# OPPO-Mente-Lab/PEA-Diffusion

Hardware: AMD Instinct MI355X
Metric: training images/sec (SDXL 1024px bf16, adapter-only bwd) (higher is better)
Workload: dtype bf16

## Files before the change

### pea_diffusion_amd/csrc/api_ops.hip

```cpp
#include <stdarg.h>
#include <string.h>

#include "../../include/pea_hip.h"
#include "pea_kernels.h"

static thread_local char g_err[512] = "";
void pea_set_error(const char* fmt, ...) {
  va_list ap;
  va_start(ap, fmt);
  vsnprintf(g_err, sizeof(g_err), fmt, ap);
  va_end(ap);
}

static bf16* g_zero_page = nullptr;
int pea_zero_page(const bf16** out) {
  if (!g_zero_page) {
    HIPCHK(hipMalloc((void**)&g_zero_page, 256));
    HIPCHK(hipMemset(g_zero_page, 0, 256));
  }
  *out = g_zero_page;
  return PEA_OK;
}

template <class P = AttnP>
static P attn_operands(const void* Q, int ldq, const void* K, int ldk, const void* V, int ldv, const void* O, int ldo,
                       const float* lse, int B, int H, int Sq, int Skv, float scale, int nd, int q_prescaled = 0) {
  AttnP p;
  memset(&p, 0, sizeof(p));
  p.Q = (const bf16*)Q; p.K = (const bf16*)K; p.V = (const bf16*)V; p.ldq = ldq; p.ldk = ldk; p.ldv = ldv;
  p.O = (bf16*)O; p.ldo = ldo; p.lse = (float*)lse; p.B = B; p.H = H; p.Sq = Sq; p.Skv = Skv; p.scale = scale; p.nd = nd;
  p.q_prescaled = q_prescaled;
  return attn_feature_p<P>(p);
}
static int attention_fwd_impl(const void* Q, int ldq, const void* K, int ldk, const void* V, int ldv, void* O, int ldo,
                              float* lse, int B, int H, int Sq, int Skv, float scale, int nd, int q_prescaled, void* stream) {
  return launch_attention_fwd(attn_operands(Q, ldq, K, ldk, V, ldv, O, ldo, lse, B, H, Sq, Skv, scale, nd, q_prescaled), (hipStream_t)stream);
}
static int attention_bwd_impl(const void* Q, int ldq, const void* K, int ldk, const void* V, int ldv, const void* O,
                              int ldo, const void* dO, int lddo, const float* lse, float* delta, void* dQ, int lddq,
                              void* dK, int lddk, void* dV, int lddv, int B, int H, int Sq, int Skv, float scale,
                              int accum_dq, int accum_dkv, int nd, void* scratch, int q_prescaled, const int* kv_len,
                              void* stream) {
  AttnP p = attn_operands(Q, ldq, K, ldk, V, ldv, O, ldo, lse, B, H, Sq, Skv, scale, nd);
  p.dO = (const bf16*)dO; p.lddo = lddo; p.delta = delta;
  p.dQ = (bf16*)dQ; p.lddq = lddq; p.dK = (bf16*)dK; p.lddk = lddk; p.dV = (bf16*)dV; p.lddv = lddv;
  p.accum_dq = accum_dq; p.accum_dkv = accum_dkv; p.dkv_part = (float*)scratch;
  p.q_prescaled = q_prescaled; p.kv_len = kv_len;
  return launch_attention_bwd(p, (hipStream_t)stream);
}

extern "C" {

const char* pea_last_error(void) { return g_err; }
int pea_version(void) { return 100; }
int pea_device_count(void) {
  int n = 0;
  if (hipGetDeviceCount(&n) != hipSuccess) return 0;
  return n;
}

int pea_op_gemm(const void* A, int lda, const void* W, int ldw, void* C, int ldc, int M, int N, int K, float alpha,
                const float* bias, const void* rowvec, int ldrv, int rows_per_batch, int act, void* preact,
                int ldpre, const void* res, int ldres, int out_f32, int accum_f32, void* stream) {
  GemmP p;
  memset(&p, 0, sizeof(p));
  p.mode = 0;
  p.A = (const bf16*)A; p.lda = lda; p.W = (const bf16*)W; p.ldw = ldw; p.C = C; p.ldc = ldc;
  p.M = M; p.N = N; p.K = K; p.alpha = alpha; p.bias = bias;
  p.rowvec = (const bf16*)rowvec; p.ldrv = ldrv; p.rows_per_batch = rows_per_batch > 0 ? rows_per_batch : 1;
  p.act = act; p.preact = (bf16*)preact; p.ldpre = ldpre; p.res = (const bf16*)res; p.ldres = ldres;
  p.out_f32 = out_f32; p.accum_f32 = accum_f32;
  return launch_gemm(p, (hipStream_t)stream);
}

int pea_op_gemm_qscale(const void* A, int lda, const void* W, int ldw, void* C, int ldc, int M, int N, int K, const float* bias,
                       int qscale_cols, float qscale, void* stream) {
  GemmP p;
  memset(&p, 0, sizeof(p));
  p.A = (const bf16*)A; p.lda = lda; p.W = (const bf16*)W; p.ldw = ldw; p.C = C; p.ldc = ldc;
  p.M = M; p.N = N; p.K = K; p.alpha = 1.f; p.bias = bias; p.rows_per_batch = 1;
  p.qscale_cols = qscale_cols; p.qscale = qscale;
  return launch_gemm(p, (hipStream_t)stream);
}

int pea_op_gemm_geglu_bwd(const void* A, int lda, const void* W, int ldw, const void* pre, int ldpre, void* C, int ldc,
                          int M, int N, int K, int form, void* stream) {
  GemmP p;
  memset(&p, 0, sizeof(p));
  p.A = (const bf16*)A; p.lda = lda; p.W = (const bf16*)W; p.ldw = ldw; p.C = C; p.ldc = ldc;
  p.M = M; p.N = N; p.K = K; p.alpha = 1.f; p.rows_per_batch = 1;
  p.gbwd_pre = (const bf16*)pre; p.ldgp = ldpre; p.gbwd_form = form;
  return launch_gemm(p, (hipStream_t)stream);
}

int pea_op_gemm_geglu(const void* A, int lda, const void* W, int ldw, const float* bias, void* y, void* stash, int M, int N,
                      int K, int stash_grad, int stash_rows, void* stream) {
  GemmP p;
  memset(&p, 0, sizeof(p));
  p.A = (const bf16*)A; p.lda = lda; p.W = (const bf16*)W; p.ldw = ldw; p.bias = bias;
  p.M = M; p.N = N; p.K = K; p.alpha = 1.f; p.rows_per_batch = 1;
  p.geglu_y = (bf16*)y; p.ldy = N / 2; p.C = stash; p.ldc = N; p.stash_grad = stash_grad; p.stash_rows = stash_rows;
  return launch_gemm(p, (hipStream_t)stream);
}

int pea_op_ln_linear(const void* x, const float* gamma, const float* beta, const void* W, const float* bias, void* y,
                     void* geglu_y, int M, int N, int K, float eps, void* Wf, float* svec, float* tvec, float* stats,
                     void* stream) {
  hipStream_t st = (hipStream_t)stream;
  int rc = launch_layernorm_stats((const bf16*)x, stats, M, K, eps, st);
  if (rc) return rc;
  rc = launch_ln_fold((const bf16*)W, K, gamma, beta, bias, (bf16*)Wf, svec, tvec, N, K, st);
  if (rc) return rc;
  GemmP p;
  memset(&p, 0, sizeof(p));
  p.A = (const bf16*)x; p.lda = K; p.W = (const bf16*)Wf; p.ldw = K; p.M = M; p.N = N; p.K = K; p.alpha = 1.f;
  p.bias = tvec; p.rows_per_batch = 1; p.ln_stats = stats; p.ln_s = svec;
  if (geglu_y) { p.geglu_y = (bf16*)geglu_y; p.ldy = N / 2; p.C = y; p.ldc = N; }
  else { p.C = y; p.ldc = N; }
  return launch_gemm(p, st);
}

int pea_op_conv3x3(const void* x, const void* w, void* y, int B, int Hs, int Ws, int Cin, int Cout, int stride,
                   int upsample2x, int transposed2, const float* bias, const void* rowvec, int ldrv,
                   const void* res, void* stream) {
// ... 374 lines not shown
```

### pea_diffusion_amd/csrc/gemm.hip

```cpp
#include <stdint.h>
#include <stdlib.h>

#include <type_traits>

#include "pea_kernels.h"

#define BK 64
constexpr int GEMM_ILV_M = 1;
constexpr int GEMM_ILV_HEAD = 4;

__device__ __forceinline__ int swz_off(int row, int chunk) { return row * 128 + ((chunk ^ ((row >> 1) & 7)) << 4); }

#ifdef PEA_GEMM_PROBES
#define PEA_PROBE(bit) (p.debug & (bit))
#else
#define PEA_PROBE(bit) false
#endif

template <int N>
__device__ __forceinline__ void wait_vmcnt() {
  static_assert(N >= 0 && N < 64, "vmcnt is a 6-bit counter");
  asm volatile("s_waitcnt vmcnt(%0)" ::"n"(N) : "memory");
}

// ... 1560 lines not shown
    SHAPECHK((span < whole ? span : whole) <= 0x7f000000LL, "gemm: one row tile of A spans %lld bytes (limit 0x7f000000)", span);
    SHAPECHK((long long)p0.N * p0.ldw * 2 <= 0x7fffffffLL, "gemm: W of %d x %d exceeds the 2 GB buffer range", p0.N, p0.ldw);
  }
  {
    double fl = 2.0 * p0.M * (double)p0.N * p0.K * (p0.parity ? 0.25 : 1.0);
    double by = 2.0 * ((double)p0.M * p0.N + (double)p0.N * p0.K + (p0.mode ? (double)p0.M * p0.K / (p0.kside == 2 ? 4.0 : (p0.kside == 4 ? 4.0 : 9.0)) : (double)p0.M * p0.K));
    if (g_prof_on) { g_prof_tag[0] = p0.M; g_prof_tag[1] = p0.N; g_prof_tag[2] = p0.K; g_prof_tag[3] = (p0.res ? 1 : 0) | (p0.bias ? 2 : 0) | (p0.rowvec ? 4 : 0); }
    PROF_BEGIN(p0.mode ? 1 : 0, fl, by, stream);
  }
  const GemmEnv& env = gemm_env();
  GemmP p = p_in;
  p.debug = g_gemm_debug;
  if (g_dbg_pf_ptr) { p.pf_ptr = g_dbg_pf_ptr; p.pf_bytes = g_dbg_pf_bytes; g_dbg_pf_ptr = nullptr; }
  if (!env.pf_on || p.pf_bytes <= 0) { p.pf_ptr = nullptr; p.pf_bytes = 0; }
  if (p.pf_bytes > env.pf_max) p.pf_bytes = env.pf_max;
  SHAPECHK(p.qscale_cols % 16 == 0 && p.qscale_cols >= 0 && p.qscale_cols <= p.N && (!p.qscale_cols || (!p.act && !p.geglu_y && !p.gbwd_pre && p.ksplit <= 1)),
           "gemm: qscale_cols=%d must be a multiple of 16 within N, on a plain (no activation / GEGLU / split-K) epilogue", p.qscale_cols);
  if (!g_num_cus) HIPCHK(gemm_query_cus());
  const GemmDecision d = gemm_decide(p, g_num_cus, g_gemm_variant, env);
  p.epi_fast = d.epi_fast;
  if (p.ksplit > 1) {
    SHAPECHK(p.out_f32 && !p.accum_f32 && !p.bias && !p.res && !p.rowvec && !p.preact && p.act == 0 && p.mode == 0,
             "gemm: split-K writes plain fp32 partials");
  }
  if (p.gbwd_pre) {
    SHAPECHK(p.epi_fast && p.mode == 0 && !p.res && !p.rowvec && !p.bias && !p.geglu_y && !p.ln_stats && p.ldgp % 8 == 0 &&
                 p.ldc >= 2 * p.N && (((unsigned long long)p.gbwd_pre & 15) == 0),
             "gemm: the fused GEGLU backward needs the batched-load epilogue (bf16 [M][2N] output, no bias / residual / row vector)");
  } else if (p.ln_stats) {
    SHAPECHK(p.epi_fast && p.ln_s && p.alpha == 1.f && p.mode == 0 && !p.res && !p.rowvec,
             "gemm: the folded-LayerNorm epilogue needs the batched-load epilogue (bf16 output, no activation / residual)");
  }
  int rc = PEA_OK;
  switch (d.inst) {
#define X(id, fn, cg, rf, gen, ...) \
    case GEMM_V##id: rc = p.mode == 0 ? fn<0, __VA_ARGS__>(p, stream) : fn<1, __VA_ARGS__>(p, stream); break;
    GEMM_TABLE(X)
#undef X
    case GEMM_GBWD_256: rc = launch_lcp<0, 256, 160, 4, 2, 4, 3, 0, 0, 3>(p, stream); break;
    case GEMM_GBWD_128: rc = launch_lcp<0, 128, 160, 4, 2, 4, 3, 0, 0, 3>(p, stream); break;
    case GEMM_GBWD_64: rc = launch_lcp<0, 64, 160, 2, 2, 4, 4, 0, 0, 3>(p, stream); break;
    case GEMM_LNF_256: rc = launch_lcp<0, 256, 160, 4, 2, 4, 3, 0, 0, 2>(p, stream); break;
    case GEMM_LNF_LC256: rc = launch_lc<0, 256, 160, 4, 2, 4, 3, false, true, 1, true>(p, stream); break;
    case GEMM_LNF_128: rc = launch_lcp<0, 128, 160, 4, 2, 4, 3, 0, 0, 2>(p, stream); break;
    case GEMM_LNF_64: rc = launch_lcp<0, 64, 160, 2, 2, 4, 4, 0, 0, 2>(p, stream); break;
    case GEMM_LNF_LC128: rc = launch_lc<0, 128, 160, 4, 2, 4, 3, false, true, 1, true>(p, stream); break;
  }
  PROF_END(stream);
  if (rc != PEA_OK) return rc;
  HIPCHK(hipGetLastError());
  return PEA_OK;
}

__global__ __launch_bounds__(256) void conv_in_kernel(const float* __restrict__ x, const float* __restrict__ w,
                                                      const float* __restrict__ bias, bf16* __restrict__ y, int B,
                                                      int Cin, int H, int W, int Cout, int pix_per_block, int ldy,
                                                      int silu) {
  extern __shared__ __attribute__((aligned(16))) char cism[];
  float* wl = (float*)cism;
  const int K = Cin * 9;
  for (int i = threadIdx.x; i < K * Cout; i += blockDim.x) {
    const int co = i / K, k = i - co * K;
    wl[k * Cout + co] = w[i];
  }
  __syncthreads();
  const int nchunk = Cout / 8;
  const int ppb = blockDim.x / nchunk;
  const int ck = threadIdx.x % nchunk, pl = threadIdx.x / nchunk;
  if (pl >= ppb) return;
  const int c0 = ck * 8;
  float bs[8];
#pragma unroll
  for (int j = 0; j < 8; ++j) bs[j] = bias[c0 + j];
  const long long npix = (long long)B * H * W;
  const long long p0 = (long long)blockIdx.x * pix_per_block;
  const long long p1 = p0 + pix_per_block < npix ? p0 + pix_per_block : npix;
  for (long long pix = p0 + pl; pix < p1; pix += ppb) {
    const int xw = (int)(pix % W), yh = (int)((pix / W) % H), b = (int)(pix / ((long long)W * H));
    float acc[8];
#pragma unroll
    for (int j = 0; j < 8; ++j) acc[j] = bs[j];
    for (int ci = 0; ci < Cin; ++ci)
#pragma unroll
      for (int ky = 0; ky < 3; ++ky) {
        const int iy = yh + ky - 1;
#pragma unroll
        for (int kx = 0; kx < 3; ++kx) {
          const int ix = xw + kx - 1;
          const bool ok = (unsigned)iy < (unsigned)H && (unsigned)ix < (unsigned)W;
          const float v = ok ? x[(((long long)b * Cin + ci) * H + iy) * W + ix] : 0.f;
          const float* wr = wl + (ci * 9 + ky * 3 + kx) * Cout + c0;
          const f32x4 w0 = *(const f32x4*)wr, w1 = *(const f32x4*)(wr + 4);
#pragma unroll
          for (int j = 0; j < 4; ++j) {
            acc[j] += v * w0[j];
            acc[4 + j] += v * w1[j];
          }
        }
      }
    bf16x8 o;
#pragma unroll
    for (int j = 0; j < 8; ++j) o[j] = (bf16)(silu ? siluf_(acc[j]) : acc[j]);
    *(bf16x8*)(y + pix * ldy + c0) = o;
  }
}

// ... 371 lines not shown
```

### pea_diffusion_amd/csrc/norm.hip

```cpp
#include "pea_kernels.h"
#ifndef PEA_LN_WT
#define PEA_LN_WT 1
#endif

#define GN_MAX_GROUPS 64

template <int BWD>
__global__ void gn_stats_kernel(const bf16* __restrict__ x, const bf16* __restrict__ dy,
                                const float* __restrict__ gamma, const float* __restrict__ beta,
                                const float* __restrict__ stats, float* __restrict__ partial, int HW, int C,
                                int groups, int pix_per_block, int silu) {
  extern __shared__ __attribute__((aligned(16))) char gsm[];
  const int nchunk = C / 8;
  const int ppb = blockDim.x / nchunk;
  const int tid = threadIdx.x;
  const int b = blockIdx.y;
  const int cpg = C / groups;
  float* tsum = (float*)gsm;
  float* csum = tsum + ppb * nchunk * 16;
  const int ck = tid % nchunk, pl = tid / nchunk;
  float s1[8], s2[8];
#pragma unroll
  for (int j = 0; j < 8; ++j) s1[j] = s2[j] = 0.f;
  if (pl < ppb) {
// ... 179 lines not shown
    for (int k = 0; k < K; ++k) red[wave][k] = (double)v[k];
  }
  __syncthreads();
#pragma unroll
  for (int k = 0; k < K; ++k) {
    double a = 0.0;
    for (int w = 0; w < nw; ++w) a += red[w][k];
    out[k] = a;
  }
  __syncthreads();
}

__device__ __forceinline__ float gn_lo(uint32_t r) { return __builtin_bit_cast(float, r << 16); }
__device__ __forceinline__ float gn_hi(uint32_t r) { return __builtin_bit_cast(float, r & 0xffff0000u); }
__device__ __forceinline__ uint32_t gn_pack(float a, float b) {
  bf16x2 v;
  v[0] = (bf16)a; v[1] = (bf16)b;
  return __builtin_bit_cast(uint32_t, v);
}
template <int W> struct GnRaw;
template <> struct GnRaw<4> { typedef uint4 T; };
template <> struct GnRaw<2> { typedef uint2 T; };
template <int W>
__device__ __forceinline__ void gn_load(uint32_t (&r)[W], const bf16* p) {
  const typename GnRaw<W>::T v = *(const typename GnRaw<W>::T*)p;
  r[0] = v.x; r[1] = v.y;
  if constexpr (W == 4) { r[2] = v.z; r[3] = v.w; }
}
template <int W>
__device__ __forceinline__ void gn_store(bf16* p, const uint32_t (&r)[W]) {
  typename GnRaw<W>::T v;
  v.x = r[0]; v.y = r[1];
  if constexpr (W == 4) { v.z = r[2]; v.w = r[3]; }
  *(typename GnRaw<W>::T*)p = v;
}
template <int N, int W>
__device__ __forceinline__ void gn_pin(uint32_t (&r)[N][W]) {
#pragma unroll
  for (int i = 0; i < N; ++i)
#pragma unroll
    for (int w = 0; w < W; ++w) asm volatile("" : "+v"(r[i][w]));
}

template <int W>
__device__ __forceinline__ void gn_chain(float& dep, uint32_t (&a)[W], uint32_t (&b)[W]) {
  if constexpr (W == 4) asm volatile("" : "+v"(dep), "+v"(a[0]), "+v"(a[1]), "+v"(a[2]), "+v"(a[3]), "+v"(b[0]), "+v"(b[1]), "+v"(b[2]), "+v"(b[3]));
  else asm volatile("" : "+v"(dep), "+v"(a[0]), "+v"(a[1]), "+v"(b[0]), "+v"(b[1]));
}

template <int VEC, int NPIX, int BWD, int GW, int SILU>
__global__ __launch_bounds__((NPIX * VEC * (1 + BWD) > 128) ? 640 : 1024) void gn_fused_kernel(
    const bf16* __restrict__ x, const bf16* __restrict__ dy, const float* __restrict__ gamma,
    const float* __restrict__ beta, float* __restrict__ stats, bf16* out, const bf16* add, int HW, int C, int groups,
    int ppb, float eps) {
  constexpr int W = VEC / 2;
  __shared__ double red[16][4];
  const int cpg = C / groups, nset = groups / GW, span = GW * cpg, nvec = span / VEC;
  const int total = gridDim.x, bid = blockIdx.x;
  const int idx = (total % 8 == 0) ? (bid % 8) * (total / 8) + bid / 8 : bid;
  const int b = idx / nset, gs = idx - b * nset;
  const int tid = threadIdx.x, vk = tid % nvec, pl0 = tid / nvec;
  const bool act = pl0 < ppb;
  const int pl = act ? pl0 : 0;
  const int c0 = gs * span + vk * VEC;
  const long long sbase = (long long)b * HW * C;
  const long long istep = (long long)ppb * C;
  const unsigned toff = (unsigned)pl * (unsigned)C + (unsigned)c0;
  bool hi[VEC];
#pragma unroll
  for (int j = 0; j < VEC; ++j) hi[j] = GW == 2 && (vk * VEC + j) >= cpg;
  uint32_t xr[NPIX][W];
  uint32_t dr[BWD ? NPIX : 1][W];
#pragma unroll
  for (int i = 0; i < NPIX; ++i) {
    gn_load<W>(xr[i], x + sbase + i * istep + toff);
    if (BWD) gn_load<W>(dr[i], dy + sbase + i * istep + toff);
  }
#define GN_X(i, j) (((j) & 1) ? gn_hi(xr[i][(j) >> 1]) : gn_lo(xr[i][(j) >> 1]))
#define GN_D(i, j) (((j) & 1) ? gn_hi(dr[i][(j) >> 1]) : gn_lo(dr[i][(j) >> 1]))
#define GN_SEL(j, a0, a1) ((GW == 2 && hi[j]) ? (a1) : (a0))
  const double count = (double)HW * cpg;
  const long long sg = (long long)b * groups + gs * GW;
  if (!BWD) {
    float s[2] = {0.f, 0.f};
#pragma unroll
    for (int i = 0; i < NPIX; ++i)
#pragma unroll
      for (int j = 0; j < VEC; ++j) {
        const float v = GN_X(i, j);
        if (GW == 2 && hi[j]) s[1] += v; else s[0] += v;
      }
    if (!act) s[0] = s[1] = 0.f;
    double m[2];
    gn_block_sum<GW>(s, red, m);
    gn_pin(xr);
    const float mean0 = (float)(m[0] / count), mean1 = GW == 2 ? (float)(m[1] / count) : 0.f;
    s[0] = s[1] = 0.f;
#pragma unroll
    for (int i = 0; i < NPIX; ++i)
#pragma unroll
      for (int j = 0; j < VEC; ++j) {
        const float d = GN_X(i, j) - GN_SEL(j, mean0, mean1);
        if (GW == 2 && hi[j]) s[1] += d * d; else s[0] += d * d;
      }
    if (!act) s[0] = s[1] = 0.f;
    double q[2];
    gn_block_sum<GW>(s, red, q);
    gn_pin(xr);
    const float rstd0 = (float)(1.0 / sqrt(q[0] / count + (double)eps));
    const float rstd1 = GW == 2 ? (float)(1.0 / sqrt(q[1] / count + (double)eps)) : 0.f;
    if (tid == 0) {
      stats[sg * 2] = mean0; stats[sg * 2 + 1] = rstd0;
// ... 1 lines not shown
    }
    if (!act) return;
    float sc[VEC], sh[VEC];
#pragma unroll
    for (int j = 0; j < VEC; ++j) {
      sc[j] = GN_SEL(j, rstd0, rstd1) * gamma[c0 + j];
      sh[j] = beta[c0 + j] - GN_SEL(j, mean0, mean1) * sc[j];
    }
#pragma unroll
    for (int i = 0; i < NPIX; ++i) {
      uint32_t o[W];
#pragma unroll
      for (int w = 0; w < W; ++w) {
        float v0 = GN_X(i, 2 * w) * sc[2 * w] + sh[2 * w], v1 = GN_X(i, 2 * w + 1) * sc[2 * w + 1] + sh[2 * w + 1];
        if (SILU) { v0 = siluf_(v0); v1 = siluf_(v1); }
        o[w] = gn_pack(v0, v1);
      }
      gn_store<W>(out + sbase + i * istep + toff, o);
    }
  } else {
    const float mean0 = stats[sg * 2], rstd0 = stats[sg * 2 + 1];
    const float mean1 = GW == 2 ? stats[sg * 2 + 2] : 0.f, rstd1 = GW == 2 ? stats[sg * 2 + 3] : 0.f;
    float gm[VEC], bt[VEC];
#pragma unroll
    for (int j = 0; j < VEC; ++j) { gm[j] = gamma[c0 + j]; bt[j] = beta[c0 + j]; }
    float s[2 * GW];
#pragma unroll
    for (int k = 0; k < 2 * GW; ++k) s[k] = 0.f;
#pragma unroll
    for (int i = 0; i < NPIX; ++i) {
#pragma unroll
      for (int j = 0; j < VEC; ++j) {
        const float xh = (GN_X(i, j) - GN_SEL(j, mean0, mean1)) * GN_SEL(j, rstd0, rstd1);
        float d = GN_D(i, j);
        if (SILU) d *= silu_grad(xh * gm[j] + bt[j]);
        d *= gm[j];
        if (GW == 2 && hi[j]) { s[1] += d; s[3] += d * xh; } else { s[0] += d; s[GW] += d * xh; }
      }
      if (i + 1 < NPIX) gn_chain<W>(s[GW], xr[i + 1], dr[i + 1]);
    }
    if (!act) {
#pragma unroll
      for (int k = 0; k < 2 * GW; ++k) s[k] = 0.f;
    }
    double r[2 * GW];
    gn_block_sum<2 * GW>(s, red, r);
    gn_pin(xr);
    gn_pin(dr);
    if (!act) return;
    const float S10 = (float)(r[0] / count), S20 = (float)(r[GW] / count);
    const float S11 = GW == 2 ? (float)(r[1] / count) : 0.f, S21 = GW == 2 ? (float)(r[2 * GW - 1] / count) : 0.f;
#pragma unroll
    for (int i = 0; i < NPIX; ++i) {
      uint32_t o[W];
      if (add) gn_load<W>(o, add + sbase + i * istep + toff);
#pragma unroll
      for (int w = 0; w < W; ++w) {
        float rr[2];
#pragma unroll
        for (int h = 0; h < 2; ++h) {
          const int j = 2 * w + h;
          const float rs = GN_SEL(j, rstd0, rstd1);
          const float xh = (GN_X(i, j) - GN_SEL(j, mean0, mean1)) * rs;
          float d = GN_D(i, j);
          if (SILU) d *= silu_grad(xh * gm[j] + bt[j]);
          d *= gm[j];
          rr[h] = rs * (d - GN_SEL(j, S10, S11) - xh * GN_SEL(j, S20, S21));
          if (add) rr[h] += h ? gn_hi(o[w]) : gn_lo(o[w]);
        }
        o[w] = gn_pack(rr[0], rr[1]);
      }
      if (i + 1 < NPIX) {
        float dep = __builtin_bit_cast(float, o[W - 1]);
        gn_chain<W>(dep, xr[i + 1], dr[i + 1]);
        o[W - 1] = __builtin_bit_cast(uint32_t, dep);
      }
      gn_store<W>(out + sbase + i * istep + toff, o);
    }
  }
#undef GN_X
#undef GN_D
#undef GN_SEL
}

struct GnFused { int vec, npix, gw, threads, ppb; };
static bool gn_fused_geometry(int HW, int C, int groups, int bwd, GnFused* f) {
  static const bool off = getenv("PEA_GN_UNFUSED") != nullptr;
  if (off) return false;
  const int cpg = C / groups;
  if (cpg % 8 == 0) { f->vec = 8; f->gw = 1; }
  else if (cpg % 4 == 0) { f->vec = 4; f->gw = 1; }
  else if (cpg % 2 == 0 && groups % 2 == 0) { f->vec = 4; f->gw = 2; }
  else return false;
  const int nvec = f->gw * cpg / f->vec;
  for (int npix = 8; npix <= 32; npix *= 2) {
    if (HW % npix) continue;
    const int regs = npix * f->vec / 2 * (1 + bwd);
    if (regs > 128) return false;
    const int maxt = regs > 64 ? 640 : 1024;
    const int thr = nvec * (HW / npix);
    if (thr > maxt) continue;
    f->npix = npix; f->ppb = HW / npix; f->threads = (thr + 63) / 64 * 64;
    return true;
  }
  return false;
}

template <int BWD>
static void gn_fused_launch(const GnFused& f, int blocks, hipStream_t s, const bf16* x, const bf16* dy, const float* gamma,
                            const float* beta, float* stats, bf16* out, const bf16* add, int HW, int C, int groups, float eps,
                            int silu) {
#define GN_S(V, N, G, S) hipLaunchKernelGGL((gn_fused_kernel<V, N, BWD, G, S>), dim3(blocks), dim3(f.threads), 0, s, x, dy, gamma, beta, \
                                            stats, out, add, HW, C, groups, f.ppb, eps)
#define GN_G(V, N, G) do { if (silu) GN_S(V, N, G, 1); else GN_S(V, N, G, 0); } while (0)
#define GN_F(V, N) do { if (f.gw == 2) GN_G(V, N, 2); else GN_G(V, N, 1); } while (0)
  if (f.vec == 8) {
    switch (f.npix) { case 8: GN_F(8, 8); break; case 16: GN_F(8, 16); break; default: GN_F(8, 32); break; }
  } else {
    switch (f.npix) { case 8: GN_F(4, 8); break; case 16: GN_F(4, 16); break; default: GN_F(4, 32); break; }
  }
#undef GN_S
#undef GN_G
#undef GN_F
}

static int gn_geometry(int HW, int C, int* threads, int* ppblk, int* nblk, size_t* lds) {
  const int nchunk = C / 8;
  if (nchunk > 1024) return -1;
  int ppb = 256 / nchunk;
  if (ppb < 1) ppb = 1;
  *threads = nchunk * ppb;
  int per = ppb * 16;
  if (per > HW) per = HW;
  *ppblk = per;
  *nblk = cdiv(HW, per);
  *lds = (size_t)(*threads) * 16 * 4 + (size_t)2 * C * 4;
  return 0;
}

size_t groupnorm_scratch_bytes(int B, int HW, int C, int groups) {
  int threads, ppblk, nblk;
  size_t lds;
  if (gn_geometry(HW, C, &threads, &ppblk, &nblk, &lds)) return 0;
  return ((size_t)B * nblk * groups * 2 + (size_t)B * groups * 2) * sizeof(float) + 256;
}

int launch_groupnorm_fwd(const bf16* x, const float* gamma, const float* beta, bf16* y, float* stats,
                         double* scratch, int B, int HW, int C, int groups, float eps, int silu, hipStream_t s) {
  SHAPECHK(C % 8 == 0 && C % groups == 0 && groups <= GN_MAX_GROUPS, "groupnorm: C=%d groups=%d", C, groups);
  int threads, ppblk, nblk;
  size_t lds;
  SHAPECHK(gn_geometry(HW, C, &threads, &ppblk, &nblk, &lds) == 0, "groupnorm: C=%d too wide", C);
  SHAPECHK(threads >= groups, "groupnorm: C=%d too narrow for %d groups", C, groups);
  float* partial = (float*)scratch;
  PROF_BEGIN(4, 0.0, 2.0 * 2.0 * B * (double)HW * C, s);
  GnFused f;
  if (gn_fused_geometry(HW, C, groups, 0, &f)) {
    gn_fused_launch<0>(f, B * (groups / f.gw), s, x, nullptr, gamma, beta, stats, y, nullptr, HW, C, groups, eps, silu);
    PROF_END(s);
    HIPCHK(hipGetLastError());
    return PEA_OK;
  }
  hipLaunchKernelGGL(gn_stats_kernel<0>, dim3(nblk, B), dim3(threads), lds, s, x, nullptr, nullptr, nullptr, nullptr,
                     partial, HW, C, groups, ppblk, 0);
  hipLaunchKernelGGL(gn_finalize_kernel, dim3(B * groups), dim3(64), 0, s, partial, stats, B * groups, groups, nblk,
                     (double)HW * (C / groups), eps, 0);
  hipLaunchKernelGGL(gn_apply_kernel, dim3(nblk, B), dim3(threads), 0, s, x, gamma, beta, stats, y, HW, C, groups,
                     silu, ppblk);
  PROF_END(s);
  HIPCHK(hipGetLastError());
  return PEA_OK;
}

int launch_groupnorm_bwd(const bf16* x, const bf16* dy, const float* gamma, const float* beta, const float* stats,
                         bf16* dx, double* scratch, int B, int HW, int C, int groups, int silu, const bf16* add,
                         hipStream_t s) {
  SHAPECHK(C % 8 == 0 && C % groups == 0 && groups <= GN_MAX_GROUPS, "groupnorm: C=%d groups=%d", C, groups);
  int threads, ppblk, nblk;
  size_t lds;
  SHAPECHK(gn_geometry(HW, C, &threads, &ppblk, &nblk, &lds) == 0, "groupnorm: C=%d too wide", C);
  SHAPECHK(threads >= groups, "groupnorm: C=%d too narrow for %d groups", C, groups);
  float* partial = (float*)scratch;
  float* sums = partial + (size_t)B * nblk * groups * 2;
  PROF_BEGIN(4, 0.0, 2.0 * (add ? 4.0 : 3.0) * B * (double)HW * C, s);
  GnFused f;
  if (gn_fused_geometry(HW, C, groups, 1, &f)) {
    gn_fused_launch<1>(f, B * (groups / f.gw), s, x, dy, gamma, beta, const_cast<float*>(stats), dx, add, HW, C, groups, 0.f, silu);
    PROF_END(s);
    HIPCHK(hipGetLastError());
    return PEA_OK;
  }
  hipLaunchKernelGGL(gn_stats_kernel<1>, dim3(nblk, B), dim3(threads), lds, s, x, dy, gamma, beta, stats, partial, HW,
                     C, groups, ppblk, silu);
  hipLaunchKernelGGL(gn_finalize_kernel, dim3(B * groups), dim3(64), 0, s, partial, sums, B * groups, groups, nblk,
                     (double)HW * (C / groups), 0.f, 1);
  hipLaunchKernelGGL(gn_bwd_apply_kernel, dim3(nblk, B), dim3(threads), 0, s, x, dy, gamma, beta, stats, sums, dx, HW,
                     C, groups, silu, add, ppblk);
  PROF_END(s);
  HIPCHK(hipGetLastError());
  return PEA_OK;
}

#define LN_MAXCH 8

#define LN_NR 2
template <int NCH, bool STATS_ONLY = false>
__global__ __launch_bounds__(256) void ln_fwd_kernel(const bf16* __restrict__ x, const float* __restrict__ gamma,
                                                     const float* __restrict__ beta, bf16* __restrict__ y,
                                                     float* __restrict__ stats, int R, int C, float eps) {
  const int lane = threadIdx.x & 63;
  const int row0 = (blockIdx.x * 4 + (threadIdx.x >> 6)) * LN_NR;
  if (row0 >= R) return;
  const int nchunk = C / 8;
  bf16x8 v[LN_NR][NCH];
#pragma unroll
  for (int r = 0; r < LN_NR; ++r) {
    const int row = min(row0 + r, R - 1);
#pragma unroll
    for (int i = 0; i < NCH; ++i) {
      const int ck = min(lane + 64 * i, nchunk - 1);
      v[r][i] = *(const bf16x8*)(x + (long long)row * C + ck * 8);
    }
  }
  f32x4 g0[STATS_ONLY ? 1 : NCH], g1[STATS_ONLY ? 1 : NCH], b0[STATS_ONLY ? 1 : NCH], b1[STATS_ONLY ? 1 : NCH];
  if constexpr (!STATS_ONLY) {
#pragma unroll
    for (int i = 0; i < NCH; ++i) {
      const int ck = min(lane + 64 * i, nchunk - 1);
      g0[i] = *(const f32x4*)(gamma + ck * 8); g1[i] = *(const f32x4*)(gamma + ck * 8 + 4);
      b0[i] = *(const f32x4*)(beta + ck * 8); b1[i] = *(const f32x4*)(beta + ck * 8 + 4);
    }
  }
  float mean[LN_NR], rstd[LN_NR];
#pragma unroll
  for (int r = 0; r < LN_NR; ++r) {
    float s = 0.f;
#pragma unroll
    for (int i = 0; i < NCH; ++i)
      if (lane + 64 * i < nchunk)
#pragma unroll
// ... 290 lines not shown
```

### pea_diffusion_amd/csrc/pea_kernels.h

```cpp
#pragma once
#include "pea_common.h"

struct GemmP {
  int mode;
  const bf16* A; int lda;
  const bf16* W; int ldw;
  void* C; int ldc; int out_f32;
  int accum_f32;
  int M, N, K;
  float alpha;
  const float* bias;
  const bf16* rowvec; int ldrv; int rows_per_batch;
  int act;
  bf16* preact; int ldpre;
  const bf16* res; int ldres;
  int Hs, Ws, Cin, Ho, Wo;
  int stride;
  int pad_off;
  int shift;
  int parity;
  int kside;
  int pad_dx;
  int pix;
  const bf16* zeros;
  int debug;
  bf16* geglu_y; int ldy;
  int geglu_tanh;
  int stash_rows;
  int stash_grad;
  int ksplit; long long split_stride;
  int epi_fast;
  const float* ln_stats; const float* ln_s;
  const bf16* gbwd_pre; int ldgp;
  int qscale_cols; float qscale;
  int gbwd_form;
  const void* pf_ptr; long long pf_bytes;
};
int launch_splitk_reduce(const float* part, int nsplit, long long stride, bf16* out, int ldo, int M, int N, int accum,
                         hipStream_t s);
int launch_gemm(const GemmP& p, hipStream_t stream);

int launch_conv_in(const float* x, const float* w, const float* bias, bf16* y, int B, int Cin, int H, int W,
                   int Cout, hipStream_t s, int ldy = 0, int silu = 0);
int launch_conv_in_gather(const float* lat, const float* mask, const float* masked, const float* w, const float* bias, bf16* y,
                          int B, int C, int lat_b, int cond_b, int H, int W, int Cout, hipStream_t s, int ldy = 0);
int launch_conv_out(const bf16* x, const float* w, const float* bias, float* y, int B, int Cin, int H, int W,
                    int Cout, hipStream_t s);
int launch_conv_out_dgrad(const float* dy, const float* w, bf16* dx, int B, int Cin, int H, int W, int Cout,
                          hipStream_t s);

int launch_groupnorm_fwd(const bf16* x, const float* gamma, const float* beta, bf16* y, float* stats,
                         double* scratch, int B, int HW, int C, int groups, float eps, int silu, hipStream_t s);
int launch_groupnorm_bwd(const bf16* x, const bf16* dy, const float* gamma, const float* beta, const float* stats,
                         bf16* dx, double* scratch, int B, int HW, int C, int groups, int silu, const bf16* add,
                         hipStream_t s);
int launch_layernorm_fwd(const bf16* x, const float* gamma, const float* beta, bf16* y, float* stats, int R, int C,
                         float eps, hipStream_t s);
int launch_rmsnorm_fwd(const bf16* x, const float* gamma, bf16* y, int R, int C, float eps, hipStream_t s);
int launch_layernorm_fwd_f32(const float* x, const float* gamma, const float* beta, float* y, int R, int C, float eps,
                             hipStream_t s);
int launch_layernorm_stats(const bf16* x, float* stats, int R, int C, float eps, hipStream_t s);
int launch_ln_fold(const bf16* W, int ldw, const float* gamma, const float* beta, const float* bias, bf16* Wf, float* svec,
                   float* tvec, int N, int K, hipStream_t s);
int launch_layernorm_bwd(const bf16* x, const bf16* dy, const float* gamma, const float* stats, bf16* dx,
                         float* dgamma, float* dbeta, int R, int C, const bf16* add, hipStream_t s);

struct AttnP {
  const bf16 *Q, *K, *V; int ldq, ldk, ldv;
  bf16* O; int ldo;
  float* lse;
  int B, H, Sq, Skv;
  float scale;
  const bf16* dO; int lddo;
  bf16 *dQ, *dK, *dV; int lddq, lddk, lddv;
  float* delta;
  int accum_dq, accum_dkv;
  float* dkv_part; int nsplit;
  int nd;
  int causal;
  const int* kv_len;
  int q_prescaled;
  const float* bias;
  const bf16 *K2, *V2; int ldk2, ldv2, Skv2;
  float scale2;
  int nset; int set_end[4]; float set_w[4]; int k2_brows;
  const float* set_mask[4]; long long set_mstride[4];
};
int attention_bwd_nsplit(int B, int H, int Sq, int Skv);
size_t attention_bwd_scratch_bytes(int B, int H, int Sq, int Skv, int nd = 1);
int launch_attention_fwd(const AttnP& p, hipStream_t s);
int launch_attention_fwd_fewq(const AttnP& p, hipStream_t s);
int launch_attention_bwd(const AttnP& p, hipStream_t s);
struct AttnRegionsP {
// ... 210 lines not shown
```

### pea_diffusion_amd/csrc/tape.hip

```cpp
#include <stdlib.h>

#include <algorithm>

#include "model.h"

int Tape::alloc() {
  tag_q_prescale();
  for (const Op& o : ops) {
    const int in[5] = {o.a, o.kind == OP_LINEAR || o.kind == OP_EMBED ? -1 : o.b, o.kind == OP_LINEAR || o.kind == OP_EMBED ? -1 : o.c, o.res, o.rv};
    for (int k = 0; k < 5; ++k) {
      if (in[k] < 0 || in[k] >= (int)tn.size() || !tn[in[k]].d2s) continue;
      SHAPECHK(o.kind == OP_CONCAT && k == 0 && o.a != o.b, "tape: op kind %d reads a depth-to-space tensor", o.kind);
    }
  }
  size_t off = 0;
  size_t max_numel = 0;
  if (owns_weights) {
    for (FusedMat& f : fused) {
      f.off_w = off; off += al256((size_t)f.N * f.K * 2);
      if (f.need_wt) { f.off_wt = off; off += al256((size_t)f.N * f.K * 2); }
      if (f.has_bias) { f.off_bias = off; off += al256((size_t)f.N * 4); }
    }
    for (WSlot& s : slots) {
      max_numel = std::max(max_numel, (size_t)s.numel);
// ... 473 lines not shown
int Tape::gemm(GemmP& p, hipStream_t s) {
  if (WSeq* q = wseq_cur) {
    const long long bytes = (p.ldw == p.K && p.ksplit <= 1) ? (long long)p.N * p.K * 2 : 0;
    if (!q->ready) q->w.push_back({(const void*)p.W, bytes});
    else {
      const size_t i = q->pos++;
      if (i >= q->w.size() || q->w[i].first != (const void*)p.W) { q->ready = false; q->w.clear(); wseq_cur = nullptr; }
      else {
        if (i + 1 < q->w.size()) {
          const Tape* ow = weights_owner ? weights_owner : this;
          const char* t = (const char*)q->w[i + 1].first;
          const long long nb = q->w[i + 1].second;
          if (ow->warena && t >= ow->warena && t + nb <= ow->warena + ow->wbytes) { p.pf_ptr = t; p.pf_bytes = nb; }
          else { q->ready = false; q->w.clear(); wseq_cur = nullptr; }
        }
      }
    }
  }
  return launch_gemm(p, s);
}

int Tape::exec_ops(size_t begin, size_t end, bool skip_cached, hipStream_t s) {
  RC(ensure_acts());
  for (size_t oi = begin; oi < end; ++oi) {
    Op& o = ops[oi];
    if (skip_cached && ce_valid && (int)oi >= ce_begin && (int)oi < ce_end) continue;
    switch (o.kind) {
      case OP_TEMB: {
        Tn& out = tn[o.out];
        if (o.src == 0) RC(launch_timestep_embed(t_in, out.d, B, o.p0, s));
        else RC(launch_timestep_embed(tid_in, out.d, B * 6, o.p0, s));
        break;
      }
      case OP_LINEAR: {
        Tn &a = tn[o.a], &out = tn[o.out];
        GemmP p; fill_gemm(p);
        p.A = a.d; p.lda = a.cols; p.M = (int)a.rows; p.K = a.cols; p.N = out.cols;
        if (o.fused >= 0) { FusedMat& f = fused[o.fused]; p.W = f.w; p.ldw = f.K; p.bias = f.bias; }
        else { WSlot& w = slots[o.w]; p.W = w.w; p.ldw = w.ldw; p.bias = o.bias >= 0 ? slots[o.bias].f32 : nullptr; }
        p.C = out.d; p.ldc = out.cols; p.act = o.p2;
        p.qscale_cols = o.qs_cols; p.qscale = o.qs;
        if (o.p3 == 3) {
          p.N = 2 * out.cols; p.geglu_y = out.d; p.ldy = out.cols; p.geglu_tanh = o.p1;
          p.C = o.c >= 0 ? tn[o.c].d : nullptr; p.ldc = 2 * out.cols;
          if (bwd_batch > 0) p.stash_rows = (int)(out.rows / B * bwd_batch);
          p.stash_grad = o.stash_form = geglu_stash_form(o);
        }
        if (o.res >= 0) { p.res = tn[o.res].d; p.ldres = tn[o.res].cols; }
        if (o.fold >= 0) {
          const LnFold& f = folds[o.fold];
          p.A = tn[ops[f.ln_op].a].d; p.W = f.wf; p.ldw = f.K; p.bias = f.t;
          p.ln_stats = ops[f.ln_op].aux; p.ln_s = f.s;
        }
        RC(gemm(p, s));
        break;
      }
      case OP_ATTN_MAT: {
        Tn &q = tn[o.a], &k = tn[o.b], &v = tn[o.c], &out = tn[o.out];
        const int HW = q.H * q.W, C = q.cols;
        for (int b = 0; b < B; ++b) {
          const long long off = (long long)b * HW * C;
          GemmP p; fill_gemm(p);
          p.A = q.d + off; p.lda = C; p.M = HW; p.K = C; p.W = k.d + off; p.ldw = C; p.N = HW; p.C = am_scores; p.ldc = HW;
          RC(launch_gemm(p, s));
          RC(launch_softmax_rows(am_scores, HW, HW, HW, o.f0, s));
          RC(launch_transpose_bf16(v.d + off, am_vt, HW, C, HW, s));
          GemmP r; fill_gemm(r);
          r.A = am_scores; r.lda = HW; r.M = HW; r.K = HW; r.W = am_vt; r.ldw = HW; r.N = C; r.C = out.d + off; r.ldc = C;
          RC(launch_gemm(r, s));
        }
        break;
      }
      case OP_EMBED: {
        SHAPECHK(ids_in != nullptr, "text encoder: no input ids");
        Tn& out = tn[o.out];
        RC(launch_embed_tokens(ids_in, slots[o.w].w,
                               o.bias >= 0 ? slots[o.bias].w + (long long)tcfg.pos_offset * out.cols : nullptr,
                               o.c >= 0 ? slots[o.c].w : nullptr, out.d, B, L, out.cols, tcfg.vocab, s));
        break;
      }
      case OP_VIS_EMBED: {
        Tn& out = tn[o.out];
        RC(launch_vision_embed(tn[o.a].d, slots[o.w].f32, slots[o.bias].w, slots[o.p0].f32, slots[o.p1].f32, out.d, B, L, out.cols,
                               o.f0, s));
        break;
      }
      case OP_CLS_ROW:
        RC(launch_copy2d(tn[o.a].d, L * tn[o.a].cols, tn[o.out].d, tn[o.out].cols, B, tn[o.out].cols, 0, s));
        break;
      case OP_GATHER_EOS:
        RC(launch_gather_eos(ids_in, tn[o.a].d, tn[o.out].d, B, L, tn[o.a].cols, tcfg.eos_id, s));
        break;
      case OP_ADD:
        RC(launch_add(tn[o.a].d, tn[o.b].d, tn[o.out].d, tn[o.out].rows * tn[o.out].cols, s));
        break;
      case OP_SILU:
        RC(launch_silu_fwd(tn[o.a].d, tn[o.out].d, tn[o.a].rows * tn[o.a].cols, s));
        break;
      case OP_CONCAT:
        if (fu_on && (o.p0 == 1 || o.p0 == 2)) {
          const Tn &a = tn[o.a], &b = tn[o.b];
          const float fs = fu_s[o.p0 - 1], fb = fu_b[o.p0 - 1];
          if (fs != 1.f) RC(launch_freeu_coef(b.d, a.B, a.H, a.W, b.cols, fu_buf, (float*)((char*)fu_buf + fu_coef_bytes), s));
          RC(launch_concat2_freeu(a.d, a.cols, b.d, b.cols, fu_buf, tn[o.out].d, a.B, a.H, a.W, fs, fb, s, a.d2s ? a.H : 0,
                                  a.d2s ? a.W : 0));
          break;
        }
// ... 142 lines not shown
      out.gw = true;
    }
    RC(materialize(out));
    if (!out.gw) continue;
    switch (o.kind) {
      case OP_LINEAR: {
        Tn& a = tn[o.a];
        if (a.rg && o.p3 == 2) {
          FusedMat& f = fused[o.fused];
          GemmP p; fill_gemm(p);
          p.A = out.g; p.lda = out.cols; p.M = (int)rb(out); p.K = out.cols; p.N = a.cols;
          p.W = f.wt; p.ldw = f.N; p.C = kv_part; p.ldc = a.cols; p.out_f32 = 1;
          p.ksplit = kv_nsplit; p.split_stride = rb(out) * a.cols;
          RC(gemm(p, s));
          RC(materialize(a));
          RC(launch_splitk_reduce(kv_part, kv_nsplit, p.split_stride, a.g, a.cols, (int)rb(a), a.cols, a.gw, s));
          a.gw = true;
          break;
        }
        if (a.rg && o.p3 == 3) {
          Tn& hg = tn[o.c];
          SHAPECHK(o.stash_form == 1, "unet: GEGLU op %d has no stash from a forward pass", oi);
          if (dpre_of != o.out) RC(launch_geglu_bwd_il(hg.d, out.g, geglu_tmp, rb(out), out.cols, s));
          dpre_of = -1;
          WSlot& w = slots[o.w];
          GemmP p; fill_gemm(p);
          p.A = geglu_tmp; p.lda = hg.cols; p.M = (int)rb(out); p.K = hg.cols; p.N = a.cols;
          p.W = w.wt; p.ldw = w.ldwt; p.C = a.g; p.ldc = a.cols;
          SHAPECHK(p.W != nullptr, "unet: dgrad weights missing for op %d", oi);
          if (const bf16* ad = addend(a)) { p.res = ad; p.ldres = a.cols; }
          RC(gemm(p, s));
          a.gw = true;
          break;
        }
        if (a.rg) {
          GemmP p; fill_gemm(p);
          p.A = out.g; p.lda = out.cols; p.M = (int)rb(out); p.K = out.cols; p.N = a.cols;
          if (o.fused >= 0) { FusedMat& f = fused[o.fused]; p.W = f.wt; p.ldw = f.N; }
          else { WSlot& w = slots[o.w]; p.W = w.wt; p.ldw = w.ldwt; }
          SHAPECHK(p.W != nullptr, "unet: dgrad weights missing for op %d", oi);
          const Op* prev = oi > 0 ? &ops[oi - 1] : nullptr;
          if (g_geglu_bwd_fused && prev && prev->kind == OP_LINEAR && prev->p3 == 3 && prev->out == o.a && prev->c >= 0 &&
              tn[prev->a].rg && !a.gw && !a.gpend && geglu_tmp && a.cols % 16 == 0) {
            Tn& hg = tn[prev->c];
            SHAPECHK(prev->stash_form >= 0, "unet: GEGLU op %d has no stash from a forward pass", oi - 1);
            p.gbwd_pre = hg.d; p.ldgp = hg.cols; p.gbwd_form = prev->stash_form;
            p.C = geglu_tmp; p.ldc = hg.cols;
            RC(gemm(p, s));
            a.gw = true;
            dpre_of = o.a;
          } else {
            p.C = a.g; p.ldc = a.cols;
            if (const bf16* ad = addend(a)) { p.res = ad; p.ldres = a.cols; }
            RC(gemm(p, s));
            a.gw = true;
          }
        }
        if (o.res >= 0 && tn[o.res].rg) RC(pass_on(out, tn[o.res]));
        break;
      }
      case OP_SILU: {
        Tn& a = tn[o.a];
        if (a.rg) { RC(materialize(a)); RC(launch_silu_bwd(a.d, out.g, a.g, rb(a) * a.cols, a.gw, s)); a.gw = true; }
        break;
      }
      case OP_CONCAT: {
        Tn &a = tn[o.a], &b = tn[o.b];
        if (o.a == o.b) {
          if (a.rg) {
            RC(materialize(a));
            RC(launch_split2(out.g, a.cols, b.cols, a.g, a.gw, nullptr, false, rb(a), s));
            RC(launch_split2(out.g, a.cols, b.cols, nullptr, false, a.g, true, rb(a), s));
            a.gw = true;
          }
          break;
        }
        if (a.rg) RC(materialize(a));
        if (b.rg) RC(materialize(b));
        RC(launch_split2(out.g, a.cols, b.cols, a.rg ? a.g : nullptr, a.gw, b.rg ? b.g : nullptr, b.gw, rb(a), s,
                         a.d2s ? a.H : 0, a.d2s ? a.W : 0));
        if (a.rg) a.gw = true;
        if (b.rg) b.gw = true;
        break;
      }
      case OP_CONV3: {
        Tn& a = tn[o.a];
        if (a.rg) {
          WSlot& w = slots[o.w];
          SHAPECHK(w.wt != nullptr, "unet: conv dgrad weights missing for %s", w.name.c_str());
          GemmP p; fill_gemm(p);
          p.mode = 1; p.A = out.g; p.W = w.wt; p.ldw = w.ldwt; p.Hs = out.H; p.Ws = out.W; p.Cin = out.cols;
          p.N = a.cols; p.K = 9 * out.cols; p.zeros = zeros; p.stride = 1;
          if (o.p1 == 2) {
            p.W = w.wt; p.ldw = w.ldwt; p.Hs = a.H; p.Ws = a.W; p.pix = 4 * out.cols; p.kside = 4; p.K = 16 * out.cols;
            p.pad_off = 1; p.Ho = a.H; p.Wo = a.W; p.M = (int)rb(a); p.C = a.g; p.ldc = a.cols;
            if (const bf16* ad = addend(a)) { p.res = ad; p.ldres = a.cols; }
            RC(gemm(p, s));
          } else if (o.p1) {
            p.Ho = out.H; p.Wo = out.W; p.M = (int)rb(out); p.C = ups_tmp; p.ldc = a.cols;
            RC(gemm(p, s));
            RC(materialize(a));
            RC(launch_sumpool2(ups_tmp, a.g, Bb, a.H, a.W, a.cols, a.gw, s));
          } else {
            if (o.p0 == 2) { p.shift = 1; p.parity = 1; }
            p.Ho = a.H; p.Wo = a.W; p.M = (int)rb(a); p.C = a.g; p.ldc = a.cols;
            if (const bf16* ad = addend(a)) { p.res = ad; p.ldres = a.cols; }
            RC(gemm(p, s));
// ... 61 lines not shown
```

Before: 41.30.

## Add skinny-M linear kernel and split GroupNorm backward across more blocks

Adds a dedicated GEMV-style kernel for linears with very few rows (M<=64, e.g. per-batch timestep/text embedding projections). It splits N across blocks and K across threads, then reduces through shared memory and DPP, instead of using the tiled GEMM that wastes most of its tile on tiny M. The tape's forward and dgrad linear paths route to it when rows equal the batch size. Separately, the fused GroupNorm backward kernel can now split each slab's pixel loop across up to four blocks when the output is not aliased, so more CUs are occupied when there are few slabs. Split blocks each recompute the slab statistics.

```diff
diff --git a/pea_diffusion_amd/csrc/api_ops.hip b/pea_diffusion_amd/csrc/api_ops.hip
--- a/pea_diffusion_amd/csrc/api_ops.hip
+++ b/pea_diffusion_amd/csrc/api_ops.hip
@@ -70,6 +70,7 @@
   p.rowvec = (const bf16*)rowvec; p.ldrv = ldrv; p.rows_per_batch = rows_per_batch > 0 ? rows_per_batch : 1;
   p.act = act; p.preact = (bf16*)preact; p.ldpre = ldpre; p.res = (const bf16*)res; p.ldres = ldres;
   p.out_f32 = out_f32; p.accum_f32 = accum_f32;
+  if (linear_is_skinny(p)) return launch_linear_skinny(p, (hipStream_t)stream);
   return launch_gemm(p, (hipStream_t)stream);
 }
 
diff --git a/pea_diffusion_amd/csrc/gemm.hip b/pea_diffusion_amd/csrc/gemm.hip
--- a/pea_diffusion_amd/csrc/gemm.hip
+++ b/pea_diffusion_amd/csrc/gemm.hip
@@ -1636,6 +1636,96 @@
   return PEA_OK;
 }
 
+#define SK_TN 4
+#define SK_THREADS 256
+#define SK_MAX_ROWS 64
+template <int MR>
+__global__ __launch_bounds__(SK_THREADS) void skinny_linear_kernel(const bf16* __restrict__ A, int lda,
+                                                                   const bf16* __restrict__ W, int ldw, bf16* C, int ldc,
+                                                                   int M, int N, int K, float alpha,
+                                                                   const float* __restrict__ bias, int act, const bf16* res,
+                                                                   int ldres) {
+  constexpr int NOUT = MR * SK_TN;
+  static_assert(NOUT * 8 <= SK_THREADS && SK_TN == 4, "skinny linear: one 8-lane group per output, column = output & 3");
+  __shared__ float red[NOUT][SK_THREADS];
+  const int tid = threadIdx.x;
+  const int n0 = blockIdx.x * SK_TN;
+  const bf16* wrow = W + (long long)n0 * ldw;
+  for (int m0 = 0; m0 < M; m0 += MR) {
+    const bf16* arow[MR];
+#pragma unroll
+    for (int r = 0; r < MR; ++r) arow[r] = A + (long long)(m0 + r < M ? m0 + r : M - 1) * lda;
+    float acc[MR][SK_TN];
+#pragma unroll
+    for (int r = 0; r < MR; ++r)
+#pragma unroll
+      for (int c = 0; c < SK_TN; ++c) acc[r][c] = 0.f;
+    for (int k = tid * 8; k < K; k += SK_THREADS * 8) {
+      bf16x8 w[SK_TN], a[MR];
+#pragma unroll
+      for (int c = 0; c < SK_TN; ++c) w[c] = *(const bf16x8*)(wrow + (long long)c * ldw + k);
+#pragma unroll
+      for (int r = 0; r < MR; ++r) a[r] = *(const bf16x8*)(arow[r] + k);
+#pragma unroll
+      for (int r = 0; r < MR; ++r)
+#pragma unroll
+        for (int c = 0; c < SK_TN; ++c)
+#pragma unroll
+          for (int j = 0; j < 8; ++j) acc[r][c] = fmaf((float)a[r][j], (float)w[c][j], acc[r][c]);
+    }
+#pragma unroll
+    for (int r = 0; r < MR; ++r)
+#pragma unroll
+      for (int c = 0; c < SK_TN; ++c) red[r * SK_TN + c][tid] = acc[r][c];
+    __syncthreads();
+    const int o = tid >> 3, sg = tid & 7;
+    float v = 0.f;
+    if (o < NOUT) {
+#pragma unroll 8
+      for (int q = 0; q < 32; ++q) v += red[o][sg * 32 + ((q + tid) & 31)];
+    }
+    v += dpp_move<0xB1>(v);
+    v += dpp_move<0x4E>(v);
+    v += dpp_move<0x141>(v);
+    const int m = m0 + (o >> 2), n = n0 + (o & 3);
+    if (sg == 0 && o < NOUT && m < M) {
+      v *= alpha;
+      if (bias) v += bias[n];
+      if (act == 1) v = gelu_erf(v);
+      else if (act == 2) v = siluf_(v);
+      else if (act == 3) v = v * sigmoidf_(1.702f * v);
+      if (res) v += (float)res[(long long)m * ldres + n];
+      C[(long long)m * ldc + n] = (bf16)v;
+    }
+    __syncthreads();
+  }
+}
+
+bool linear_is_skinny(const GemmP& p) {
+  auto al = [](const void* q, unsigned a) { return ((unsigned long long)q & (a - 1)) == 0; };
+  return p.mode == 0 && p.M > 0 && p.M <= SK_MAX_ROWS && p.N > 0 && p.N % SK_TN == 0 && p.K > 0 && p.K % BK == 0 &&
+         p.lda % 8 == 0 && p.ldw % 8 == 0 && p.ldc % 4 == 0 && al(p.A, 16) && al(p.W, 16) && p.C && al(p.C, 8) &&
+         (!p.bias || al(p.bias, 16)) && (!p.res || (p.ldres % 4 == 0 && al(p.res, 8))) && p.act >= 0 && p.act <= 3 &&
+         !p.out_f32 && !p.accum_f32 && !p.rowvec && !p.preact && !p.geglu_y && !p.gbwd_pre && !p.ln_stats && !p.qscale_cols &&
+         p.ksplit <= 1 && g_gemm_variant < 0 && !g_gemm_debug;
+}
+
+int launch_linear_skinny(const GemmP& p, hipStream_t stream) {
+  SHAPECHK(linear_is_skinny(p), "skinny linear: M=%d N=%d K=%d is not a plain thin linear", p.M, p.N, p.K);
+  if (g_prof_on) { g_prof_tag[0] = p.M; g_prof_tag[1] = p.N; g_prof_tag[2] = p.K; g_prof_tag[3] = (p.res ? 1 : 0) | (p.bias ? 2 : 0); }
+  PROF_BEGIN(0, 2.0 * p.M * (double)p.N * p.K, 2.0 * ((double)p.M * p.N + (double)p.N * p.K + (double)p.M * p.K), stream);
+  const dim3 grid(p.N / SK_TN), block(SK_THREADS);
+  if (p.M <= 4)
+    hipLaunchKernelGGL(skinny_linear_kernel<4>, grid, block, 0, stream, p.A, p.lda, p.W, p.ldw, (bf16*)p.C, p.ldc, p.M, p.N, p.K,
+                       p.alpha, p.bias, p.act, p.res, p.ldres);
+  else
+    hipLaunchKernelGGL(skinny_linear_kernel<8>, grid, block, 0, stream, p.A, p.lda, p.W, p.ldw, (bf16*)p.C, p.ldc, p.M, p.N, p.K,
+                       p.alpha, p.bias, p.act, p.res, p.ldres);
+  PROF_END(stream);
+  HIPCHK(hipGetLastError());
+  return PEA_OK;
+}
+
 __global__ __launch_bounds__(256) void conv_in_kernel(const float* __restrict__ x, const float* __restrict__ w,
                                                       const float* __restrict__ bias, bf16* __restrict__ y, int B,
                                                       int Cin, int H, int W, int Cout, int pix_per_block, int ldy,
diff --git a/pea_diffusion_amd/csrc/norm.hip b/pea_diffusion_amd/csrc/norm.hip
--- a/pea_diffusion_amd/csrc/norm.hip
+++ b/pea_diffusion_amd/csrc/norm.hip
@@ -255,12 +255,13 @@
 __global__ __launch_bounds__((NPIX * VEC * (1 + BWD) > 128) ? 640 : 1024) void gn_fused_kernel(
     const bf16* __restrict__ x, const bf16* __restrict__ dy, const float* __restrict__ gamma,
     const float* __restrict__ beta, float* __restrict__ stats, bf16* out, const bf16* add, int HW, int C, int groups,
-    int ppb, float eps) {
+    int ppb, float eps, int pmask) {
   constexpr int W = VEC / 2;
   __shared__ double red[16][4];
   const int cpg = C / groups, nset = groups / GW, span = GW * cpg, nvec = span / VEC;
   const int total = gridDim.x, bid = blockIdx.x;
-  const int idx = (total % 8 == 0) ? (bid % 8) * (total / 8) + bid / 8 : bid;
+  const int vid = (total % 8 == 0) ? (bid % 8) * (total / 8) + bid / 8 : bid;
+  const int idx = BWD ? vid / (pmask + 1) : vid, part = BWD ? vid & pmask : 0;
   const int b = idx / nset, gs = idx - b * nset;
   const int tid = threadIdx.x, vk = tid % nvec, pl0 = tid / nvec;
   const bool act = pl0 < ppb;
@@ -368,6 +369,7 @@
     const float S11 = GW == 2 ? (float)(r[1] / count) : 0.f, S21 = GW == 2 ? (float)(r[2 * GW - 1] / count) : 0.f;
 #pragma unroll
     for (int i = 0; i < NPIX; ++i) {
+      if ((i & pmask) != part) continue;
       uint32_t o[W];
       if (add) gn_load<W>(o, add + sbase + i * istep + toff);
 #pragma unroll
@@ -399,6 +401,7 @@
 #undef GN_SEL
 }
 
+#define GN_SPLIT_CUS 256
 struct GnFused { int vec, npix, gw, threads, ppb; };
 static bool gn_fused_geometry(int HW, int C, int groups, int bwd, GnFused* f) {
   static const bool off = getenv("PEA_GN_UNFUSED") != nullptr;
@@ -425,9 +428,9 @@
 template <int BWD>
 static void gn_fused_launch(const GnFused& f, int blocks, hipStream_t s, const bf16* x, const bf16* dy, const float* gamma,
                             const float* beta, float* stats, bf16* out, const bf16* add, int HW, int C, int groups, float eps,
-                            int silu) {
+                            int silu, int pmask = 0) {
 #define GN_S(V, N, G, S) hipLaunchKernelGGL((gn_fused_kernel<V, N, BWD, G, S>), dim3(blocks), dim3(f.threads), 0, s, x, dy, gamma, beta, \
-                                            stats, out, add, HW, C, groups, f.ppb, eps)
+                                            stats, out, add, HW, C, groups, f.ppb, eps, pmask)
 #define GN_G(V, N, G) do { if (silu) GN_S(V, N, G, 1); else GN_S(V, N, G, 0); } while (0)
 #define GN_F(V, N) do { if (f.gw == 2) GN_G(V, N, 2); else GN_G(V, N, 1); } while (0)
   if (f.vec == 8) {
@@ -501,7 +504,12 @@
   PROF_BEGIN(4, 0.0, 2.0 * (add ? 4.0 : 3.0) * B * (double)HW * C, s);
   GnFused f;
   if (gn_fused_geometry(HW, C, groups, 1, &f)) {
-    gn_fused_launch<1>(f, B * (groups / f.gw), s, x, dy, gamma, beta, const_cast<float*>(stats), dx, add, HW, C, groups, 0.f, silu);
+    const int slabs = B * (groups / f.gw);
+    int parts = 1;
+    if (dx != x && dx != dy)
+      while (parts < 4 && slabs * parts * 2 <= GN_SPLIT_CUS) parts *= 2;
+    gn_fused_launch<1>(f, slabs * parts, s, x, dy, gamma, beta, const_cast<float*>(stats), dx, add, HW, C, groups, 0.f, silu,
+                       parts - 1);
     PROF_END(s);
     HIPCHK(hipGetLastError());
     return PEA_OK;
diff --git a/pea_diffusion_amd/csrc/pea_kernels.h b/pea_diffusion_amd/csrc/pea_kernels.h
--- a/pea_diffusion_amd/csrc/pea_kernels.h
+++ b/pea_diffusion_amd/csrc/pea_kernels.h
@@ -39,6 +39,8 @@
 int launch_splitk_reduce(const float* part, int nsplit, long long stride, bf16* out, int ldo, int M, int N, int accum,
                          hipStream_t s);
 int launch_gemm(const GemmP& p, hipStream_t stream);
+bool linear_is_skinny(const GemmP& p);
+int launch_linear_skinny(const GemmP& p, hipStream_t stream);
 
 int launch_conv_in(const float* x, const float* w, const float* bias, bf16* y, int B, int Cin, int H, int W,
                    int Cout, hipStream_t s, int ldy = 0, int silu = 0);
diff --git a/pea_diffusion_amd/csrc/tape.hip b/pea_diffusion_amd/csrc/tape.hip
--- a/pea_diffusion_amd/csrc/tape.hip
+++ b/pea_diffusion_amd/csrc/tape.hip
@@ -549,7 +549,7 @@
           p.A = tn[ops[f.ln_op].a].d; p.W = f.wf; p.ldw = f.K; p.bias = f.t;
           p.ln_stats = ops[f.ln_op].aux; p.ln_s = f.s;
         }
-        RC(gemm(p, s));
+        RC(a.rows == B && linear_is_skinny(p) ? launch_linear_skinny(p, s) : gemm(p, s));
         break;
       }
       case OP_ATTN_MAT: {
@@ -798,7 +798,7 @@
           } else {
             p.C = a.g; p.ldc = a.cols;
             if (const bf16* ad = addend(a)) { p.res = ad; p.ldres = a.cols; }
-            RC(gemm(p, s));
+            RC(out.rows == B && linear_is_skinny(p) ? launch_linear_skinny(p, s) : gemm(p, s));
             a.gw = true;
           }
         }
```

Measured after the change: 41.58, median of 6. No clear change (+0.7%).
